# proroklab/magat_pathplanning

Hardware: AMD Instinct MI355X
Metric: agent-steps/s (batched GAT forward) (higher is better)
Workload: dtype f32 in/out, fp32-class arithmetic: convolutions + GAT maps as f16x3 split products on the 16-bit matrix cores with f32 accumulation (the encoder head too, on the layer3 kernel's pooled map; with GAT_MFMA the attention scores and the K-hop aggregation as well), MLPs on f32 MFMA

## Files before the change

include/magat_hip.h:

```cpp
#ifndef MAGAT_HIP_H
#define MAGAT_HIP_H

#include <stddef.h>
#include <stdint.h>

#ifdef __cplusplus
extern "C" {
#endif

#define MAGAT_OK 0
#define MAGAT_ERR_BAD_SHAPE (-1)
#define MAGAT_ERR_UNSUPPORTED (-2)
#define MAGAT_ERR_WORKSPACE (-3)
#define MAGAT_ERR_LAUNCH (-4)
#define MAGAT_ERR_NULL (-5)

#define MAGAT_MODE_KEYQUERY 0
#define MAGAT_MODE_GAT_MODIFIED 1
#define MAGAT_MODE_GAT_ORIGIN 2
#define MAGAT_MODE_GNN 3

int magat_abi_version(void);
int magat_build_flavor(void);
const char* magat_error_string(int code);
// ... 245 lines not shown
#define MAGAT_FORM_GAT_PACK 2
#define MAGAT_FORM_GAT_PERSIST 3
#define MAGAT_FORM_GAT_HSPLIT 4
#define MAGAT_FORM_CHAIN_PERSIST 5
#define MAGAT_FORM_HEAD_COMPRESS 6
#define MAGAT_FORM_GUARD_ONE 7
#define MAGAT_FORM_CSR_FUSED 8
#define MAGAT_FORM_GAT_MID 9
#define MAGAT_FORM_CHAIN_LAT 10
#define MAGAT_FORM_HEAD_LAT 11
#define MAGAT_FORM_GUARD_LAT 12
#define MAGAT_FORM_STEM_LAT 13
#define MAGAT_FORM_ACTIONS_TAIL 14
#define MAGAT_FORM_GNN_DENSE 15
#define MAGAT_FORMS 16
long long magat_form_count(int id);
int magat_form_reset(void);

#ifdef __cplusplus
}
#endif
#endif
```

magat_pathplanning_amd/_native.py:

```python
import ctypes
import os
import threading

PKG = os.path.dirname(os.path.abspath(__file__))
LIB_PATH = os.environ.get("MAGAT_LIB_PATH") or os.path.join(PKG, "lib", "libmagat_hip.so")

MODE_KEYQUERY = 0
MODE_GAT_MODIFIED = 1
MODE_GAT_ORIGIN = 2
MODE_GNN = 3
_MODE_IDS = {"KeyQuery": MODE_KEYQUERY, "GAT_modified": MODE_GAT_MODIFIED, "GAT_origin": MODE_GAT_ORIGIN}
TAGS = {0: "untagged", 1: "conv_first", 2: "layer1.conv1", 3: "layer1.conv2+ds", 4: "layer2.conv1",
        5: "layer2.conv2+ds", 6: "layer3.conv1", 7: "layer3.conv2+ds", 8: "head(avgpool+fc+linear)",
        9: "compressMLP", 10: "gat_maps_gemm", 11: "gat_graph", 12: "actionsMLP", 13: "head_mean",
        14: "gat_pack", 15: "gso_prepare", 16: "gat_prepare", 17: "range_guard", 18: "layer1.conv2+layer2 (fused)", 19: "gat_layer (one launch)", 20: "gso_to_csr", 21: "gat_cast", 22: "layer3 (fused, pooled)", 23: "layer1.conv2+layer2+layer3 (fused, pooled)", 25: "gnn_dense"}
TAG_ACTIONS = 12
FORMS = {"head_longk": 0, "head_splitk": 1, "gat_pack": 2, "gat_persist": 3, "gat_hsplit": 4, "chain_persist": 5,
         "head_compress": 6, "guard_one": 7, "csr_fused": 8, "gat_mid": 9, "chain_lat": 10, "head_lat": 11, "guard_lat": 12, "stem_lat": 13, "actions_tail": 14, "gnn_dense": 15}
TAG_GNN_DENSE = 25

_lock = threading.Lock()
_lib = None


class MagatNativeError(RuntimeError):
    pass


class ConvGemmDesc(ctypes.Structure):
    _fields_ = [("inp", ctypes.c_void_p), ("in2", ctypes.c_void_p), ("wt", ctypes.c_void_p),
                ("bias", ctypes.c_void_p), ("out", ctypes.c_void_p),
                ("in_pix_stride", ctypes.c_int64), ("in2_pix_stride", ctypes.c_int64),
                ("out_pix_stride", ctypes.c_int64), ("M", ctypes.c_int),
# ... 177 lines not shown
```

magat_pathplanning_amd/csrc/gat_mfma.hip:

```cpp
#include <type_traits>

#include "magat_common.h"

namespace {

typedef _Float16 f16x8 __attribute__((ext_vector_type(8)));
typedef _Float16 f16x2 __attribute__((ext_vector_type(2)));

struct GatMfmaParams {
  const float* X;
  const void* S;
  const unsigned* rmask_pre;
  const char* wfrag;
  const float* bias;
  float* Y;
  int B, N, P, ldx, ldy, concat, s_is_f64;
  int Binst;
  int hsplit;
  float* Ypre; int ldpre;
  int* range_flag;
  const float* kconst;
  int origin;
  const float* x_scale;
  long long* dbg;
// ... 67 lines not shown
    const float send = odd ? a[r0] : a[r0 + 1];
    const float recv = dpp_mov<0xB1>(send);
    a[r0] = odd ? recv : a[r0];
    a[r0 + 1] = odd ? a[r0 + 1] : recv;
  }
#pragma unroll
  for (int r0 = 0; r0 < 2; ++r0) {
    const float send = hi ? a[r0] : a[r0 + 2];
    const float recv = dpp_mov<0x4E>(send);
    a[r0] = hi ? recv : a[r0];
    a[r0 + 2] = hi ? a[r0 + 2] : recv;
  }
}

__device__ __forceinline__ uint4 lds128(const char* ptr, int coff) { return *reinterpret_cast<const uint4*>(ptr + coff); }

template <int MT, int KSI, int KT, bool CONCAT, int MODE, bool PACK = false>
__global__ __launch_bounds__(256, 1) void gat_mfma_kernel(const GatMfmaParams p) {
  extern __shared__ __align__(16) char lds[];
  static_assert(!PACK || (MT == 4 && KSI == 2), "PACK: four 32-row slots");
  constexpr int KI = 16 * KSI, SA = 2 * KI + 16;
  constexpr int KIU = PACK ? 128 : KI, SAU = 2 * KIU + 16;
  constexpr int MTS = PACK ? 1 : MT;
  constexpr float kInvScale = 1.f / 256.f;
  const int t = threadIdx.x, lane = t & 63;
  const int w = __builtin_amdgcn_readfirstlane(t >> 6);
  const int fr = lane & 31, h_ = lane >> 5;
  const int N = p.N;
  const int NR = PACK ? 128 : N;
  const int R8 = PACK ? 128 : (N + 7) & ~7;
// ... 26 lines not shown
  auto wr_load = [&](int hd_, int f) __attribute__((always_inline)) {
    int hh = hd_;
    if (f >= FPH) { hh = hd_ + 1 == hhi ? hlo : hd_ + 1; f -= FPH; }
    const int ks = f & 7;
    const char* s = f < 8 ? wl + (size_t)hh * 65536
                          : wl + (size_t)(p.P + hh * KT + (KT - 1 - (f - 8) / 8)) * 65536;
    wr[f & 3][0] = *reinterpret_cast<const uint4*>(s + ks * 2048);
    wr[f & 3][1] = *reinterpret_cast<const uint4*>(s + ks * 2048 + 1024);
  };
#pragma unroll
  for (int f = 0; f < 4; ++f) wr_load(hlo, f);

  for (int b = b0; b < p.B; b += bstride) {
    GM_STAMP(14);
    if (b != b0) GM_SYNC();
    {
      int t = threadIdx.x;
      asm volatile("" : "+v"(t));
      const int lane_ = t & 63;
      const float* Xb = p.X + (long long)b * (PACK ? 4 : 1) * N * p.ldx;
      const unsigned xst = AO + 2048;
      for (int c = w; c * 64 < NR * 32; c += 4) {
        const int ch = c * 64 + lane_;
        const int row = ch >> 5;
        const long long arow = PACK ? (long long)(row >> 5) * N + (row & 31) : row;
        const bool rok = PACK ? ((row & 31) < N && 4 * b + (row >> 5) < p.Binst) : ch < N * 32;
        const float* src = Xb + arow * p.ldx + (ch & 31) * 4;
        const unsigned m0v = __builtin_amdgcn_readfirstlane((unsigned)(uintptr_t)lds + xst + (unsigned)c * 1024u);
        if (rok) asm volatile("s_mov_b32 m0, %1\n\tglobal_load_lds_dwordx4 %0, off" ::"v"(src), "s"(m0v) : "memory", "m0");
      }
      if (!p.rmask_pre) {
        auto stage_pack = [&](auto tag) __attribute__((always_inline)) {
          typedef decltype(tag) ST;
          const int j0 = (lane_ & 31) < N ? (lane_ & 31) : N - 1;
          for (int R0 = w; R0 < 128; R0 += 32) {
            ST v0[8];
#pragma unroll
            for (int r = 0; r < 8; ++r) {
              const int R = R0 + 4 * r, sl = R >> 5, i = min(R & 31, N - 1);
              const int inst = min(4 * b + sl, p.Binst - 1);
              v0[r] = (static_cast<const ST*>(p.S) + (long long)inst * N * N)[(long long)i * N + j0];
            }
#pragma unroll
            for (int r = 0; r < 8; ++r) {
              const int R = R0 + 4 * r, sl = R >> 5, i = R & 31;
              bool f0 = sizeof(ST) == 8 ? fabs((double)v0[r]) > 1e-9 : fabsf((float)v0[r]) > 1e-9f;
              if (MODE == 1 && p.origin) f0 = fabsf((float)v0[r] + ((lane_ & 31) == i ? 1.f : 0.f)) > 1e-9f;
              const unsigned long long k0 = __ballot(f0 && lane_ < N);
              if (lane_ == 0) {
                unsigned* m = reinterpret_cast<unsigned*>(lds + MO) + 4 * R;
                m[0] = (i < N && 4 * b + sl < p.Binst) ? (unsigned)k0 : 0u; m[1] = 0u; m[2] = 0u; m[3] = 0u;
              }
            }
          }
        };
        auto stage = [&](auto tag) {
          typedef decltype(tag) ST;
          const ST* Sp = static_cast<const ST*>(p.S) + (long long)b * N * N;
          const int j0 = lane_ < N ? lane_ : N - 1, j1 = lane_ + 64 < N ? lane_ + 64 : N - 1;
          for (int i0 = w; i0 < N; i0 += 32) {
            ST v0[8], v1[8];
#pragma unroll
            for (int r = 0; r < 8; ++r) {
              const int i = i0 + 4 * r < N ? i0 + 4 * r : N - 1;
              v0[r] = Sp[(long long)i * N + j0];
              v1[r] = Sp[(long long)i * N + j1];
            }
#pragma unroll
            for (int r = 0; r < 8; ++r) {
              const int i = i0 + 4 * r;
              bool f0 = sizeof(ST) == 8 ? fabs((double)v0[r]) > 1e-9 : fabsf((float)v0[r]) > 1e-9f;
              bool f1 = sizeof(ST) == 8 ? fabs((double)v1[r]) > 1e-9 : fabsf((float)v1[r]) > 1e-9f;
              if (MODE == 1 && p.origin) {
                f0 = fabsf((float)v0[r] + (lane_ == i ? 1.f : 0.f)) > 1e-9f;
                f1 = fabsf((float)v1[r] + (lane_ + 64 == i ? 1.f : 0.f)) > 1e-9f;
              }
              const unsigned long long k0 = __ballot(f0 && lane_ < N), k1 = __ballot(f1 && lane_ + 64 < N);
              if (lane_ == 0 && i < N) {
                unsigned* m = reinterpret_cast<unsigned*>(lds + MO) + 4 * i;
                m[0] = (unsigned)k0; m[1] = (unsigned)(k0 >> 32); m[2] = (unsigned)k1; m[3] = (unsigned)(k1 >> 32);
              }
            }
          }
        };
        if constexpr (PACK) {
          if (p.s_is_f64) stage_pack(double{});
          else stage_pack(float{});
        } else {
          if (p.s_is_f64) stage(double{});
          else stage(float{});
        }
      }
      asm volatile("s_waitcnt vmcnt(0)" ::: "memory");
      GM_SYNC();
      for (int idx = t; idx < NR * 16; idx += 256) {
        const int row = idx >> 4, ch = idx & 15;
        f32x4 v0 = *reinterpret_cast<const f32x4*>(lds + xst + idx * 32);
        f32x4 v1 = *reinterpret_cast<const f32x4*>(lds + xst + idx * 32 + 16);
        if (PACK && !((row & 31) < N && 4 * b + (row >> 5) < p.Binst)) v0 = v1 = f32x4{0.f, 0.f, 0.f, 0.f};
        float xv[8] = {v0[0] * xs, v0[1] * xs, v0[2] * xs, v0[3] * xs, v1[0] * xs, v1[1] * xs, v1[2] * xs, v1[3] * xs};
        bool bad = false;
#pragma unroll
        for (int e = 0; e < 8; ++e) bad |= !(fabsf(xv[e]) <= 65504.f);
        if (bad) vmax = __builtin_inff();
        uint4 hi, lo;
        split2v(xv[0], xv[1], hi.x, lo.x, vmax);
        split2v(xv[2], xv[3], hi.y, lo.y, vmax);
        split2v(xv[4], xv[5], hi.z, lo.z, vmax);
        split2v(xv[6], xv[7], hi.w, lo.w, vmax);
        char* dst = lds + (row * 512 + ((ch ^ (row & 15)) << 4));
        *reinterpret_cast<uint4*>(dst) = hi;
        *reinterpret_cast<uint4*>(dst + 256) = lo;
      }
    }
    GM_SYNC();
    GM_STAMP(15);
    unsigned mk[4] = {0u, 0u, 0u, 0u};
    if constexpr (PACK) {
      if (fr < N && 4 * b + w < p.Binst) {
        const unsigned m = p.rmask_pre ? p.rmask_pre[((long long)(4 * b + w) * N + fr) * 4]
                                       : *reinterpret_cast<const unsigned*>(lds + MO + 16 * cw_);
        mk[0] = m >> (4 * h_);
      }
    } else if (cw_ < N) {
      const uint4 m = p.rmask_pre ? *reinterpret_cast<const uint4*>(p.rmask_pre + ((long long)b * N + cw_) * 4)
                                  : *reinterpret_cast<const uint4*>(lds + MO + 16 * cw_);
      mk[0] = m.x >> (4 * h_); mk[1] = m.y >> (4 * h_); mk[2] = m.z >> (4 * h_); mk[3] = m.w >> (4 * h_);
    }
#pragma unroll 1
// ... 386 lines not shown
              }
            }
#ifdef GM_WHATIF_NOYST
            GM_SINK(o[0]);
#else
            if (rok) *dst = o;
#endif
          }
      }
      GM_STAMP(10);
    }
  }
  if (p.range_flag && vmax > 65504.f) atomicOr(p.range_flag, 1);
}

size_t gat_mfma_lds(int N, int ksi) {
  const size_t sa = 2 * 16 * (size_t)ksi + 16, r8 = ((size_t)N + 7) & ~(size_t)7;
  return 2 * (size_t)N * 256 + 2 * r8 * sa + 2 * 128 * sa;
}
constexpr size_t kGatPackLds = 2 * 128 * 256 + 2 * 128 * 80 + 2 * 128 * 272;

int gat_mfma_class(int N) {
  if (N <= 0) return -1;
  const int c = N <= 32 ? 0 : (N <= 64 ? 1 : 2);
  const int ksi = c == 0 ? 2 : (c == 1 ? 4 : 7);
  return (N <= 16 * ksi && gat_mfma_lds(N, ksi) <= 160 * 1024) ? c : -1;
}

template <int KT, int MODE>
int launch_pack(const GatMfmaParams& p, int slot, hipStream_t st) {
// ... 21 lines not shown
int launch(const GatMfmaParams& p, int slot, hipStream_t st) {
  const size_t lds = gat_mfma_lds(p.N, KSI);
  const void* fn = p.concat ? reinterpret_cast<const void*>(&gat_mfma_kernel<MT, KSI, KT, true, MODE>)
                            : reinterpret_cast<const void*>(&gat_mfma_kernel<MT, KSI, KT, false, MODE>);
  if (magat_ensure_dyn_lds(fn, slot + (p.concat ? 0 : 6) + 12 * MODE, lds) != MAGAT_OK) return MAGAT_ERR_LAUNCH;
  int cus = 256, dev = 0;
  if (hipGetDevice(&dev) != hipSuccess ||
      hipDeviceGetAttribute(&cus, hipDeviceAttributeMultiprocessorCount, dev) != hipSuccess || cus <= 0)
    cus = 256;
  GatMfmaParams q = p;
  const long long unsplit = (long long)((p.B + cus - 1) / cus) * (12 + 36 * p.P);
  const long long split = (long long)(((long long)p.B * p.P + cus - 1) / cus) * (12 + 36);
  q.hsplit = ((p.concat || p.Ypre) && p.P > 1 && split < unsplit) ? p.P : 1;
  const long long units = q.hsplit > 1 ? (long long)p.B * p.P : p.B;
  const int blocks = (int)(units < (long long)cus * q.hsplit ? units : (long long)cus * q.hsplit);
  if (q.hsplit > 1) magat_form_note(MAGAT_FORM_GAT_HSPLIT);
  if (units > blocks) magat_form_note(MAGAT_FORM_GAT_PERSIST);
  const int pid = magat_prof_begin(MAGAT_TAG_GAT_LAYER, st);
  if (p.concat) hipLaunchKernelGGL((gat_mfma_kernel<MT, KSI, KT, true, MODE>), dim3(blocks), dim3(256), lds, st, q);
  else {
    hipLaunchKernelGGL((gat_mfma_kernel<MT, KSI, KT, false, MODE>), dim3(blocks), dim3(256), lds, st, q);
    if (q.hsplit > 1 && magat_gat_mean_launch(p.Ypre, p.Y, (long long)p.B * p.N, p.P, 128, p.ldpre, p.ldy, st) != MAGAT_OK) {
      magat_prof_end(pid, st);
      return MAGAT_ERR_LAUNCH;
    }
  }
  magat_prof_end(pid, st);
  return magat_check_launch();
}

template <int MODE>
int launch_class(const GatMfmaParams& p, int K, hipStream_t st) {
  const int cls = gat_mfma_class(p.N);
// ... 46 lines not shown
```

magat_pathplanning_amd/csrc/magat_common.h:

```cpp
#pragma once
#include <hip/hip_runtime.h>
#include <stdint.h>

#include "../../include/magat_hip.h"

typedef float f32x2 __attribute__((ext_vector_type(2)));
typedef float f32x4 __attribute__((ext_vector_type(4)));
typedef float f32x16 __attribute__((ext_vector_type(16)));

#if (defined(MAGAT_WHATIF_NO_W) || defined(MAGAT_WHATIF_NO_LDS) || defined(CSR_WHATIF_NODMA) || defined(CSR_WHATIF_NOLOOP) || defined(CSR_WHATIF_NOIDX) || defined(CSR_WHATIF_NOKLOOP) || defined(CSR_WHATIF_NOSTORE) || \
     defined(GM_WHATIF_NOQW) || defined(GM_WHATIF_NOAW) || defined(GM_WHATIF_NOYST) || defined(FUSED_WHATIF_COALESCED) || defined(FUSED_WHATIF_NOSCALAR)) && !defined(MAGAT_EXPERIMENT_BUILD)
#error "*_WHATIF_* timing switches produce wrong results: they compile only with -DMAGAT_EXPERIMENT_BUILD (see magat_common.h)"
#endif
extern "C" int magat_experiment_mark(void);
#ifdef MAGAT_EXPERIMENT_BUILD
namespace { struct MagatExperimentMark { MagatExperimentMark() { magat_experiment_mark(); } } g_magat_experiment_mark; }
#endif

#define MAGAT_WAVE 64
#define MAGAT_TILE_ROWS 128
__host__ __device__ __forceinline__ long long magat_row_off(long long m, long long ld, long long tile_stride) {
  return (m >> 7) * tile_stride + (m & 127) * ld;
}
#define MAGAT_NUM_XCD 8
// ... 37 lines not shown
                    const float* scales = nullptr, int out_gl = 0, const magat_lat_head* head = nullptr,
                    const magat_lat_guard* guard = nullptr, const magat_lat_stem* stem = nullptr);
int magat_block3(const void* in, float* out, const float* w, const float* b1, const float* b2, int M, int* range_flag,
                 hipStream_t st);
int magat_block_chain(const void* in1, const void* in2, void* out, int out_gl, long long out_pix_stride, long long out_tile,
                      const float* w, const float* bA, const float* bB, const float* bC, int M, int* range_flag,
                      hipStream_t st);
int magat_conv_direct_enabled();
int magat_conv_gemm_chain_f32(const magat_conv_gemm_desc* descs, int n, const int32_t* run_if, int tag, hipStream_t st,
                              int32_t* book = nullptr);

enum MagatOpt {
  MAGAT_OPT_ENC_CHUNK, MAGAT_OPT_CONV_SPLIT, MAGAT_OPT_CONV_PCHAIN,
  MAGAT_OPT_L1_FUSED, MAGAT_OPT_HEAD_SPLITK, MAGAT_OPT_GAT_CHUNK_MB, MAGAT_OPT_GAT_SPLIT, MAGAT_OPT_RANGE_GUARD,
  MAGAT_OPT_BLOCK_FUSED, MAGAT_OPT_CSR_TILED, MAGAT_OPT_HEAD_F16, MAGAT_OPT_GAT_MFMA, MAGAT_OPT_SKINNY, MAGAT_OPT_GAT_PACK,
  MAGAT_OPT_CONV_BNFILL, MAGAT_OPT_HEAD_COMPRESS, MAGAT_OPT_CONV_TM, MAGAT_OPT_CSR_FUSED, MAGAT_OPT_LAT_AGENTS, MAGAT_OPT_GAT_WIDE_FROM, MAGAT_OPT_COUNT
};
int magat_opt(int id);
#define MAGAT_LDS_SLOTS 192
int magat_ensure_dyn_lds(const void* func, int slot, size_t bytes);
enum MagatLdsSlot {
  MAGAT_LDS_GAT16, MAGAT_LDS_GAT32, MAGAT_LDS_GAT64, MAGAT_LDS_GAT128, MAGAT_LDS_GAT256, MAGAT_LDS_L1FUSED,
  MAGAT_LDS_SIM_GSO_T, MAGAT_LDS_SIM_GSO_F, MAGAT_LDS_SIM_MOVE, MAGAT_LDS_BLOCK_A, MAGAT_LDS_BLOCK_B, MAGAT_LDS_BLOCK_C,
  MAGAT_LDS_SIM_CONN, MAGAT_LDS_CONV_FIRST, MAGAT_LDS_CONV_FIRST11, MAGAT_LDS_GSO_STRUCT, MAGAT_LDS_CSR_TILED_A, MAGAT_LDS_CSR_TILED_B, MAGAT_LDS_CSR_TILED_A16, MAGAT_LDS_CSR_TILED_B16,
  MAGAT_LDS_CSR_TILED_A4, MAGAT_LDS_CSR_TILED_B4, MAGAT_LDS_CSR_TILED_A16_4, MAGAT_LDS_CSR_TILED_B16_4, MAGAT_LDS_BLOCK_B4, MAGAT_LDS_BLOCK_FULL, MAGAT_LDS_BLOCK_FULL_P, MAGAT_LDS_BLOCK_FULL_C, MAGAT_LDS_BLOCK_FULL_C4, MAGAT_LDS_BLOCK_FULL_C5,
  MAGAT_LDS_GATM_0,
  MAGAT_LDS_GATM_END = MAGAT_LDS_GATM_0 + 24,
  MAGAT_LDS_STEM8,
  MAGAT_LDS_GATP_0,
  MAGAT_LDS_GATP_END = MAGAT_LDS_GATP_0 + 8,
  MAGAT_LDS_GATS_0,
  MAGAT_LDS_GATS_END = MAGAT_LDS_GATS_0 + 8,
  MAGAT_LDS_CSR_FUSED_A,
  MAGAT_LDS_CSR_FUSED_B = MAGAT_LDS_CSR_FUSED_A + 3,
  MAGAT_LDS_CSR_FUSED_END = MAGAT_LDS_CSR_FUSED_B + 2,
  MAGAT_LDS_GATD_0 = MAGAT_LDS_CSR_FUSED_END,
  MAGAT_LDS_GATD_END = MAGAT_LDS_GATD_0 + 56,
  MAGAT_LDS_BLOCK_LAT, MAGAT_LDS_BLOCK_LAT_H, MAGAT_LDS_BLOCK_LAT_S,
  MAGAT_LDS_GAT_SLIM,
  MAGAT_LDS_GAT_RERUN_S, MAGAT_LDS_GAT_RERUN_S_END = MAGAT_LDS_GAT_RERUN_S + 5,
  MAGAT_LDS_GNND_0,
  MAGAT_LDS_GNND_END = MAGAT_LDS_GNND_0 + 5,
  MAGAT_LDS_END
};
static_assert(MAGAT_LDS_END <= MAGAT_LDS_SLOTS, "LDS attribute slots");

__host__ __device__ inline size_t magat_gat_f16_block_offset(int NC, int G) {
  const size_t a = (((size_t)NC * (G + 1) + 3) & ~(size_t)3) + ((size_t)3 * NC * G + 1) / 2;
  return (a + 3) & ~(size_t)3;
}

__host__ __device__ inline size_t magat_gat_frag_offset(int NC, int G) {
  return (magat_gat_f16_block_offset(NC, G) + (size_t)NC * G + 4 + 3) & ~(size_t)3;
}
__host__ __device__ inline size_t magat_gat_csr_fused_offset(int NC, int G) {
  return (magat_gat_frag_offset(NC, G) + (size_t)NC * G + 3) & ~(size_t)3;
}
// ... 109 lines not shown
```

magat_pathplanning_amd/csrc/options.hip:

```cpp
#include <atomic>
#include <cstdlib>
#include <cstring>
#include <mutex>

#include "magat_common.h"

namespace {

struct OptEntry {
  const char* name;
  int def;
};

const OptEntry kOpts[MAGAT_OPT_COUNT] = {
    {"ENC_CHUNK", 65536},
    {"CONV_SPLIT", 7},
    {"CONV_PCHAIN", 1},
    {"L1_FUSED", 2},
    {"HEAD_SPLITK", 5120},
    {"GAT_CHUNK_MB", 2048},
    {"GAT_SPLIT", 1},
    {"RANGE_GUARD", 1},
    {"BLOCK_FUSED", 2},
    {"CSR_TILED", 3},
    {"HEAD_F16", 1},
    {"GAT_MFMA", 1},
    {"SKINNY", 1},
    {"GAT_PACK", 1},
    {"CONV_BNFILL", 256},
    {"HEAD_COMPRESS", 1},
    {"CONV_TM", 2},
    {"CSR_FUSED", 1},
    {"LAT_AGENTS", 512},
    {"GAT_WIDE_FROM", 103},
};

int g_val[MAGAT_OPT_COUNT];
int g_start[MAGAT_OPT_COUNT];
std::once_flag g_once;

void init_opts() {
  for (int i = 0; i < MAGAT_OPT_COUNT; ++i) {
    g_val[i] = kOpts[i].def;
    char key[64] = "MAGAT_";
    strncat(key, kOpts[i].name, sizeof(key) - 7);
    const char* e = getenv(key);
    if (e && *e) g_val[i] = atoi(e);
    g_start[i] = g_val[i];
  }
// ... 67 lines not shown
```

magat_pathplanning_amd/csrc/profile.hip:

```cpp
#include <algorithm>
#include <atomic>
#include <mutex>
#include <vector>

#include "magat_common.h"

namespace {
struct Span {
  int tag;
  hipEvent_t a, b;
};
bool g_enabled = false;
std::vector<Span> g_pool;
size_t g_used = 0;
double g_total[MAGAT_PROF_TAGS];
long long g_count[MAGAT_PROF_TAGS];
std::mutex g_mu;
constexpr size_t kMaxSpans = 1 << 16;
}

int magat_prof_begin(int tag, hipStream_t st) {
  if (!g_enabled || tag == MAGAT_TAG_UNTAGGED) return -1;
  std::lock_guard<std::mutex> lk(g_mu);
  if (g_used >= kMaxSpans) return -1;
// ... 133 lines not shown
  if (stamps) {
    std::vector<long long> h(2 * (size_t)cus);
    if (hipMemcpy(h.data(), stamps, h.size() * sizeof(long long), hipMemcpyDeviceToHost) != hipSuccess) return MAGAT_ERR_LAUNCH;
    std::vector<double> mhz;
    for (int i = 0; i < cus; ++i)
      if (h[2 * i + 1] > 0) mhz.push_back((double)h[2 * i] / (double)h[2 * i + 1] * 100.0);
    if (mhz.empty()) return MAGAT_ERR_LAUNCH;
    std::sort(mhz.begin(), mhz.end());
    const double med = mhz[mhz.size() / 2];
    if (clock_mhz) *clock_mhz = med;
    if (per_clk) *per_clk = *tflops * 1e12 / (med * 1e6 * (double)cus * 4);
  }
  return MAGAT_OK;
}

namespace { std::atomic<long long> g_forms[MAGAT_FORMS]; }
void magat_form_note(int id) {
  if (id >= 0 && id < MAGAT_FORMS) g_forms[id].fetch_add(1, std::memory_order_relaxed);
}
extern "C" long long magat_form_count(int id) {
  if (id < 0 || id >= MAGAT_FORMS) return -1;
  return g_forms[id].load(std::memory_order_relaxed);
}
extern "C" int magat_form_reset(void) {
  for (int i = 0; i < MAGAT_FORMS; ++i) g_forms[i].store(0, std::memory_order_relaxed);
  return MAGAT_OK;
}
```

Measured before the change: 22.06 million.

## Add 512-thread paired-wavefront GAT kernel splitting map GEMM and tap aggregation

Adds a gat_pair_kernel that runs 8 wavefronts per block. Four wavefronts compute the per-head map GEMM while the other four handle the attention tap and K-hop aggregation, so the two phases can overlap within one block. The staging code is factored into a helper templated on wavefront count so both kernels share it. The kernel is enabled by default for KeyQuery concat layers. This adds register and LDS pressure and more block-level synchronisation.

```diff
diff --git a/include/magat_hip.h b/include/magat_hip.h
--- a/include/magat_hip.h
+++ b/include/magat_hip.h
@@ -283,6 +283,8 @@
 #define MAGAT_FORM_ACTIONS_TAIL 14
 #define MAGAT_FORM_GNN_DENSE 15
 #define MAGAT_FORMS 16
+#define MAGAT_FORM_GAT_PAIR 16
+#define MAGAT_FORMS_ALL 17
 long long magat_form_count(int id);
 int magat_form_reset(void);
 
diff --git a/magat_pathplanning_amd/_native.py b/magat_pathplanning_amd/_native.py
--- a/magat_pathplanning_amd/_native.py
+++ b/magat_pathplanning_amd/_native.py
@@ -16,7 +16,8 @@
         14: "gat_pack", 15: "gso_prepare", 16: "gat_prepare", 17: "range_guard", 18: "layer1.conv2+layer2 (fused)", 19: "gat_layer (one launch)", 20: "gso_to_csr", 21: "gat_cast", 22: "layer3 (fused, pooled)", 23: "layer1.conv2+layer2+layer3 (fused, pooled)", 25: "gnn_dense"}
 TAG_ACTIONS = 12
 FORMS = {"head_longk": 0, "head_splitk": 1, "gat_pack": 2, "gat_persist": 3, "gat_hsplit": 4, "chain_persist": 5,
-         "head_compress": 6, "guard_one": 7, "csr_fused": 8, "gat_mid": 9, "chain_lat": 10, "head_lat": 11, "guard_lat": 12, "stem_lat": 13, "actions_tail": 14, "gnn_dense": 15}
+         "head_compress": 6, "guard_one": 7, "csr_fused": 8, "gat_mid": 9, "chain_lat": 10, "head_lat": 11, "guard_lat": 12, "stem_lat": 13, "actions_tail": 14, "gnn_dense": 15,
+         "gat_pair": 16}
 TAG_GNN_DENSE = 25
 
 _lock = threading.Lock()
diff --git a/magat_pathplanning_amd/csrc/gat_mfma.hip b/magat_pathplanning_amd/csrc/gat_mfma.hip
--- a/magat_pathplanning_amd/csrc/gat_mfma.hip
+++ b/magat_pathplanning_amd/csrc/gat_mfma.hip
@@ -105,6 +105,110 @@
 }
 
 __device__ __forceinline__ uint4 lds128(const char* ptr, int coff) { return *reinterpret_cast<const uint4*>(ptr + coff); }
+
+template <int NW, int MODE, bool PACK>
+__device__ __forceinline__ void gm_stage_instance(const GatMfmaParams& p, char* lds, int b, int w, int N, int NR, unsigned AO,
+                                                  unsigned MO, float xs, float& vmax) {
+  {
+    int t = threadIdx.x;
+    asm volatile("" : "+v"(t));
+    const int lane_ = t & 63;
+    const float* Xb = p.X + (long long)b * (PACK ? 4 : 1) * N * p.ldx;
+    const unsigned xst = AO + 2048;
+    for (int c = w; c * 64 < NR * 32; c += NW) {
+      const int ch = c * 64 + lane_;
+      const int row = ch >> 5;
+      const long long arow = PACK ? (long long)(row >> 5) * N + (row & 31) : row;
+      const bool rok = PACK ? ((row & 31) < N && 4 * b + (row >> 5) < p.Binst) : ch < N * 32;
+      const float* src = Xb + arow * p.ldx + (ch & 31) * 4;
+      const unsigned m0v = __builtin_amdgcn_readfirstlane((unsigned)(uintptr_t)lds + xst + (unsigned)c * 1024u);
+      if (rok) asm volatile("s_mov_b32 m0, %1\n\tglobal_load_lds_dwordx4 %0, off" ::"v"(src), "s"(m0v) : "memory", "m0");
+    }
+    if (!p.rmask_pre) {
+      auto stage_pack = [&](auto tag) __attribute__((always_inline)) {
+        typedef decltype(tag) ST;
+        const int j0 = (lane_ & 31) < N ? (lane_ & 31) : N - 1;
+        for (int R0 = w; R0 < 128; R0 += 8 * NW) {
+          ST v0[8];
+#pragma unroll
+          for (int r = 0; r < 8; ++r) {
+            const int R = R0 + NW * r, sl = R >> 5, i = min(R & 31, N - 1);
+            const int inst = min(4 * b + sl, p.Binst - 1);
+            v0[r] = (static_cast<const ST*>(p.S) + (long long)inst * N * N)[(long long)i * N + j0];
+          }
+#pragma unroll
+          for (int r = 0; r < 8; ++r) {
+            const int R = R0 + NW * r, sl = R >> 5, i = R & 31;
+            bool f0 = sizeof(ST) == 8 ? fabs((double)v0[r]) > 1e-9 : fabsf((float)v0[r]) > 1e-9f;
+            if (MODE == 1 && p.origin) f0 = fabsf((float)v0[r] + ((lane_ & 31) == i ? 1.f : 0.f)) > 1e-9f;
+            const unsigned long long k0 = __ballot(f0 && lane_ < N);
+            if (lane_ == 0) {
+              unsigned* m = reinterpret_cast<unsigned*>(lds + MO) + 4 * R;
+              m[0] = (i < N && 4 * b + sl < p.Binst) ? (unsigned)k0 : 0u; m[1] = 0u; m[2] = 0u; m[3] = 0u;
+            }
+          }
+        }
+      };
+      auto stage = [&](auto tag) {
+        typedef decltype(tag) ST;
+        const ST* Sp = static_cast<const ST*>(p.S) + (long long)b * N * N;
+        const int j0 = lane_ < N ? lane_ : N - 1, j1 = lane_ + 64 < N ? lane_ + 64 : N - 1;
+        for (int i0 = w; i0 < N; i0 += 8 * NW) {
+          ST v0[8], v1[8];
+#pragma unroll
+          for (int r = 0; r < 8; ++r) {
+            const int i = i0 + NW * r < N ? i0 + NW * r : N - 1;
+            v0[r] = Sp[(long long)i * N + j0];
+            v1[r] = Sp[(long long)i * N + j1];
+          }
+#pragma unroll
+          for (int r = 0; r < 8; ++r) {
+            const int i = i0 + NW * r;
+            bool f0 = sizeof(ST) == 8 ? fabs((double)v0[r]) > 1e-9 : fabsf((float)v0[r]) > 1e-9f;
+            bool f1 = sizeof(ST) == 8 ? fabs((double)v1[r]) > 1e-9 : fabsf((float)v1[r]) > 1e-9f;
+            if (MODE == 1 && p.origin) {
+              f0 = fabsf((float)v0[r] + (lane_ == i ? 1.f : 0.f)) > 1e-9f;
+              f1 = fabsf((float)v1[r] + (lane_ + 64 == i ? 1.f : 0.f)) > 1e-9f;
+            }
+            const unsigned long long k0 = __ballot(f0 && lane_ < N), k1 = __ballot(f1 && lane_ + 64 < N);
+            if (lane_ == 0 && i < N) {
+              unsigned* m = reinterpret_cast<unsigned*>(lds + MO) + 4 * i;
+              m[0] = (unsigned)k0; m[1] = (unsigned)(k0 >> 32); m[2] = (unsigned)k1; m[3] = (unsigned)(k1 >> 32);
+            }
+          }
+        }
+      };
+      if constexpr (PACK) {
+        if (p.s_is_f64) stage_pack(double{});
+        else stage_pack(float{});
+      } else {
+        if (p.s_is_f64) stage(double{});
+        else stage(float{});
+      }
+    }
+    asm volatile("s_waitcnt vmcnt(0)" ::: "memory");
+    GM_SYNC();
+    for (int idx = t; idx < NR * 16; idx += 64 * NW) {
+      const int row = idx >> 4, ch = idx & 15;
+      f32x4 v0 = *reinterpret_cast<const f32x4*>(lds + xst + idx * 32);
+      f32x4 v1 = *reinterpret_cast<const f32x4*>(lds + xst + idx * 32 + 16);
+      if (PACK && !((row & 31) < N && 4 * b + (row >> 5) < p.Binst)) v0 = v1 = f32x4{0.f, 0.f, 0.f, 0.f};
+      float xv[8] = {v0[0] * xs, v0[1] * xs, v0[2] * xs, v0[3] * xs, v1[0] * xs, v1[1] * xs, v1[2] * xs, v1[3] * xs};
+      bool bad = false;
+#pragma unroll
+      for (int e = 0; e < 8; ++e) bad |= !(fabsf(xv[e]) <= 65504.f);
+      if (bad) vmax = __builtin_inff();
+      uint4 hi, lo;
+      split2v(xv[0], xv[1], hi.x, lo.x, vmax);
+      split2v(xv[2], xv[3], hi.y, lo.y, vmax);
+      split2v(xv[4], xv[5], hi.z, lo.z, vmax);
+      split2v(xv[6], xv[7], hi.w, lo.w, vmax);
+      char* dst = lds + (row * 512 + ((ch ^ (row & 15)) << 4));
+      *reinterpret_cast<uint4*>(dst) = hi;
+      *reinterpret_cast<uint4*>(dst + 256) = lo;
+    }
+  }
+}
 
 template <int MT, int KSI, int KT, bool CONCAT, int MODE, bool PACK = false>
 __global__ __launch_bounds__(256, 1) void gat_mfma_kernel(const GatMfmaParams p) {
@@ -161,105 +265,7 @@
   for (int b = b0; b < p.B; b += bstride) {
     GM_STAMP(14);
     if (b != b0) GM_SYNC();
-    {
-      int t = threadIdx.x;
-      asm volatile("" : "+v"(t));
-      const int lane_ = t & 63;
-      const float* Xb = p.X + (long long)b * (PACK ? 4 : 1) * N * p.ldx;
-      const unsigned xst = AO + 2048;
-      for (int c = w; c * 64 < NR * 32; c += 4) {
-        const int ch = c * 64 + lane_;
-        const int row = ch >> 5;
-        const long long arow = PACK ? (long long)(row >> 5) * N + (row & 31) : row;
-        const bool rok = PACK ? ((row & 31) < N && 4 * b + (row >> 5) < p.Binst) : ch < N * 32;
-        const float* src = Xb + arow * p.ldx + (ch & 31) * 4;
-        const unsigned m0v = __builtin_amdgcn_readfirstlane((unsigned)(uintptr_t)lds + xst + (unsigned)c * 1024u);
-        if (rok) asm volatile("s_mov_b32 m0, %1\n\tglobal_load_lds_dwordx4 %0, off" ::"v"(src), "s"(m0v) : "memory", "m0");
-      }
-      if (!p.rmask_pre) {
-        auto stage_pack = [&](auto tag) __attribute__((always_inline)) {
-          typedef decltype(tag) ST;
-          const int j0 = (lane_ & 31) < N ? (lane_ & 31) : N - 1;
-          for (int R0 = w; R0 < 128; R0 += 32) {
-            ST v0[8];
-#pragma unroll
-            for (int r = 0; r < 8; ++r) {
-              const int R = R0 + 4 * r, sl = R >> 5, i = min(R & 31, N - 1);
-              const int inst = min(4 * b + sl, p.Binst - 1);
-              v0[r] = (static_cast<const ST*>(p.S) + (long long)inst * N * N)[(long long)i * N + j0];
-            }
-#pragma unroll
-            for (int r = 0; r < 8; ++r) {
-              const int R = R0 + 4 * r, sl = R >> 5, i = R & 31;
-              bool f0 = sizeof(ST) == 8 ? fabs((double)v0[r]) > 1e-9 : fabsf((float)v0[r]) > 1e-9f;
-              if (MODE == 1 && p.origin) f0 = fabsf((float)v0[r] + ((lane_ & 31) == i ? 1.f : 0.f)) > 1e-9f;
-              const unsigned long long k0 = __ballot(f0 && lane_ < N);
-              if (lane_ == 0) {
-                unsigned* m = reinterpret_cast<unsigned*>(lds + MO) + 4 * R;
-                m[0] = (i < N && 4 * b + sl < p.Binst) ? (unsigned)k0 : 0u; m[1] = 0u; m[2] = 0u; m[3] = 0u;
-              }
-            }
-          }
-        };
-        auto stage = [&](auto tag) {
-          typedef decltype(tag) ST;
-          const ST* Sp = static_cast<const ST*>(p.S) + (long long)b * N * N;
-          const int j0 = lane_ < N ? lane_ : N - 1, j1 = lane_ + 64 < N ? lane_ + 64 : N - 1;
-          for (int i0 = w; i0 < N; i0 += 32) {
-            ST v0[8], v1[8];
-#pragma unroll
-            for (int r = 0; r < 8; ++r) {
-              const int i = i0 + 4 * r < N ? i0 + 4 * r : N - 1;
-              v0[r] = Sp[(long long)i * N + j0];
-              v1[r] = Sp[(long long)i * N + j1];
-            }
-#pragma unroll
-            for (int r = 0; r < 8; ++r) {
-              const int i = i0 + 4 * r;
-              bool f0 = sizeof(ST) == 8 ? fabs((double)v0[r]) > 1e-9 : fabsf((float)v0[r]) > 1e-9f;
-              bool f1 = sizeof(ST) == 8 ? fabs((double)v1[r]) > 1e-9 : fabsf((float)v1[r]) > 1e-9f;
-              if (MODE == 1 && p.origin) {
-                f0 = fabsf((float)v0[r] + (lane_ == i ? 1.f : 0.f)) > 1e-9f;
-                f1 = fabsf((float)v1[r] + (lane_ + 64 == i ? 1.f : 0.f)) > 1e-9f;
-              }
-              const unsigned long long k0 = __ballot(f0 && lane_ < N), k1 = __ballot(f1 && lane_ + 64 < N);
-              if (lane_ == 0 && i < N) {
-                unsigned* m = reinterpret_cast<unsigned*>(lds + MO) + 4 * i;
-                m[0] = (unsigned)k0; m[1] = (unsigned)(k0 >> 32); m[2] = (unsigned)k1; m[3] = (unsigned)(k1 >> 32);
-              }
-            }
-          }
-        };
-        if constexpr (PACK) {
-          if (p.s_is_f64) stage_pack(double{});
-          else stage_pack(float{});
-        } else {
-          if (p.s_is_f64) stage(double{});
-          else stage(float{});
-        }
-      }
-      asm volatile("s_waitcnt vmcnt(0)" ::: "memory");
-      GM_SYNC();
-      for (int idx = t; idx < NR * 16; idx += 256) {
-        const int row = idx >> 4, ch = idx & 15;
-        f32x4 v0 = *reinterpret_cast<const f32x4*>(lds + xst + idx * 32);
-        f32x4 v1 = *reinterpret_cast<const f32x4*>(lds + xst + idx * 32 + 16);
-        if (PACK && !((row & 31) < N && 4 * b + (row >> 5) < p.Binst)) v0 = v1 = f32x4{0.f, 0.f, 0.f, 0.f};
-        float xv[8] = {v0[0] * xs, v0[1] * xs, v0[2] * xs, v0[3] * xs, v1[0] * xs, v1[1] * xs, v1[2] * xs, v1[3] * xs};
-        bool bad = false;
-#pragma unroll
-        for (int e = 0; e < 8; ++e) bad |= !(fabsf(xv[e]) <= 65504.f);
-        if (bad) vmax = __builtin_inff();
-        uint4 hi, lo;
-        split2v(xv[0], xv[1], hi.x, lo.x, vmax);
-        split2v(xv[2], xv[3], hi.y, lo.y, vmax);
-        split2v(xv[4], xv[5], hi.z, lo.z, vmax);
-        split2v(xv[6], xv[7], hi.w, lo.w, vmax);
-        char* dst = lds + (row * 512 + ((ch ^ (row & 15)) << 4));
-        *reinterpret_cast<uint4*>(dst) = hi;
-        *reinterpret_cast<uint4*>(dst + 256) = lo;
-      }
-    }
+    gm_stage_instance<4, MODE, PACK>(p, lds, b, w, N, NR, AO, MO, xs, vmax);
     GM_SYNC();
     GM_STAMP(15);
     unsigned mk[4] = {0u, 0u, 0u, 0u};
@@ -676,6 +682,410 @@
   if (p.range_flag && vmax > 65504.f) atomicOr(p.range_flag, 1);
 }
 
+#ifdef MAGAT_DEBUG_HOOKS
+#define GP_STAMP(i) do { if (p.dbg && (threadIdx.x & 63) == 0) p.dbg[((long long)blockIdx.x * 4 + ((threadIdx.x >> 6) & 3)) * 16 + (i)] = (long long)__builtin_readcyclecounter(); } while (0)
+#else
+#define GP_STAMP(i) do { } while (0)
+#endif
+#define GP_VMAX() asm volatile("" : "+v"(vmax))
+template <int MT, int KSI, int KT>
+__global__ __launch_bounds__(512, 1) void gat_pair_kernel(const GatMfmaParams p) {
+  extern __shared__ __align__(16) char lds[];
+  constexpr int KI = 16 * KSI, SA = 2 * KI + 16;
+  constexpr int SAU = SA;
+  constexpr float kInvScale = 1.f / 256.f;
+  const int t = threadIdx.x, lane = t & 63;
+  const int wv = __builtin_amdgcn_readfirstlane(t >> 6);
+  const int w = wv & 3;
+  const bool tapw = wv >= 4;
+  const int fr = lane & 31, h_ = lane >> 5;
+  const int N = p.N;
+  const int NR = N, R8 = (N + 7) & ~7;
+  const unsigned AO = 512u * NR, AP = (unsigned)R8 * SA;
+  const unsigned UO = AO + 2 * AP;
+  constexpr unsigned UP = 128 * SAU;
+  const unsigned MO = AO;
+#define GP_ROWS(rsw, xsw) unsigned rsw[MT], xsw[MT]; { int l_ = lane; asm volatile("" : "+v"(l_)); _Pragma("unroll") \
+    for (int mt_ = 0; mt_ < MT; ++mt_) { const int row_ = min(32 * mt_ + (l_ & 31), N - 1); rsw[mt_] = row_ * 512; \
+      xsw[mt_] = ((l_ >> 5) ^ (row_ & 15)) << 4; } }
+  const int cw_ = 32 * w + fr;
+  auto wlo = [&]() __attribute__((always_inline)) { unsigned o = (unsigned)lane * 16u; asm volatile("" : "+v"(o)); return (unsigned)w * 16384u + o; };
+  float vmax = 0.f;
+  float xs = 1.f;
+  if (p.x_scale) xs = *p.x_scale;
+  if (xs == 0.f) xs = 1.f;
+  const float ixs = 1.f / xs;
+  const int hpw = p.P / p.hsplit, hlo = ((int)blockIdx.x % p.hsplit) * hpw, hhi = hlo + hpw;
+  const int b0 = (int)blockIdx.x / p.hsplit, bstride = (int)gridDim.x / p.hsplit;
+  uint4 wr[4][2];
+
+  if (!tapw) {
+    const bool g2_active = 32 * w < KI;
+    const float kLog2eS = 1.4426950408889634f * ixs * ixs;
+    auto wr_load = [&](int hd_, int f) __attribute__((always_inline)) {
+      int hh = hd_;
+      if (f >= 8) { hh = hd_ + 1 == hhi ? hlo : hd_ + 1; f -= 8; }
+      const char* s = p.wfrag + (wlo() + (unsigned)hh * 65536u + (unsigned)f * 2048u);
+      wr[f & 3][0] = *reinterpret_cast<const uint4*>(s);
+      wr[f & 3][1] = *reinterpret_cast<const uint4*>(s + 1024);
+    };
+#pragma unroll
+    for (int f = 0; f < 4; ++f) wr_load(hlo, f);
+    f32x16 accq[MT];
+    auto g1 = [&](int hd) __attribute__((always_inline)) {
+      GP_ROWS(rsw, xsw)
+#pragma unroll
+      for (int mt = 0; mt < MT; ++mt)
+#pragma unroll
+        for (int r = 0; r < 16; ++r) accq[mt][r] = 0.f;
+      uint4 a[MT][2];
+#pragma unroll
+      for (int mt = 0; mt < MT; ++mt) {
+        const char* ap = lds + (rsw[mt] + xsw[mt]);
+        a[mt][0] = lds128(ap, 0);
+        a[mt][1] = lds128(ap, 256);
+      }
+#pragma unroll
+      for (int ks = 0; ks < 8; ++ks) {
+#pragma unroll
+        for (int q = 0; q < 3; ++q)
+#pragma unroll
+          for (int mt = 0; mt < MT; ++mt) {
+            accq[mt] = mfma16(wr[ks & 3][q == 1 ? 1 : 0], a[mt][q == 2 ? 1 : 0], accq[mt]);
+            if (ks + 1 < 8 && q >= 1)
+              a[mt][q - 1] = lds128(lds + (rsw[mt] + (xsw[mt] ^ (unsigned)((ks + 1) << 5))), 256 * (q - 1));
+          }
+        wr_load(hd, ks + 4);
+        GM_PIN();
+      }
+    };
+    for (int b = b0; b < p.B; b += bstride) {
+      GP_STAMP(14);
+      if (b != b0) GM_SYNC();
+      gm_stage_instance<8, 0, false>(p, lds, b, wv, N, NR, AO, MO, xs, vmax);
+      GM_SYNC();
+      GP_STAMP(15);
+      unsigned mk[4] = {0u, 0u, 0u, 0u};
+      if (cw_ < N) {
+        const uint4 m = p.rmask_pre ? *reinterpret_cast<const uint4*>(p.rmask_pre + ((long long)b * N + cw_) * 4)
+                                    : *reinterpret_cast<const uint4*>(lds + MO + 16 * cw_);
+        mk[0] = m.x >> (4 * h_); mk[1] = m.y >> (4 * h_); mk[2] = m.z >> (4 * h_); mk[3] = m.w >> (4 * h_);
+      }
+      g1(hlo);
+      GP_STAMP(11);
+#pragma unroll 1
+      for (int hd = hlo; hd < hhi; ++hd) {
+        GP_STAMP(0);
+        int cw = cw_, h = h_;
+        asm volatile("" : "+v"(cw), "+v"(h));
+        if (hd > hlo) GM_SYNC();
+        GP_STAMP(1);
+        {
+          const int fr_ = cw & 31;
+          unsigned jb[MT];
+#pragma unroll
+          for (int mt = 0; mt < MT; ++mt) {
+            const int j = 32 * mt + fr_;
+            jb[mt] = UO + (unsigned)(j < R8 ? j : R8) * 512u + 8u * h;
+          }
+          unsigned qx[4];
+#pragma unroll
+          for (int q = 0; q < 4; ++q) {
+            qx[q] = (unsigned)(((4 * w + q) ^ (fr_ & 15)) << 4);
+            asm volatile("" : "+v"(qx[q]));
+          }
+#pragma unroll
+          for (int mt = 0; mt < MT; ++mt)
+#pragma unroll
+            for (int q = 0; q < 4; ++q) {
+              unsigned hq[2], lq[2];
+              const float v01[2] = {mul1(accq[mt][4 * q], kInvScale), mul1(accq[mt][4 * q + 1], kInvScale)};
+              split2v(v01[0], v01[1], hq[0], lq[0], vmax);
+              GP_VMAX();
+              const float v23[2] = {mul1(accq[mt][4 * q + 2], kInvScale), mul1(accq[mt][4 * q + 3], kInvScale)};
+              split2v(v23[0], v23[1], hq[1], lq[1], vmax);
+              GP_VMAX();
+              char* o = lds + (jb[mt] + qx[q]);
+              GM_QW(o, (uint2{hq[0], hq[1]}));
+              GM_QW(o + 256, (uint2{lq[0], lq[1]}));
+            }
+        }
+        GP_STAMP(2);
+        GM_SYNC();
+        GP_STAMP(3);
+        if (g2_active) {
+          GP_ROWS(rsw, xsw)
+          f32x16 acce[MT];
+#pragma unroll
+          for (int mt = 0; mt < MT; ++mt)
+#pragma unroll
+            for (int r = 0; r < 16; ++r) acce[mt][r] = 0.f;
+          {
+            const int rowb = min(32 * w + (cw & 31), N - 1);
+            const unsigned rswb = rowb * 512, xswb = (h ^ (rowb & 15)) << 4;
+            const char* qbase = lds + UO;
+            uint4 a[MT][2], bq[2][2];
+#pragma unroll
+            for (int mt = 0; mt < MT; ++mt) {
+              const char* ap = qbase + (rsw[mt] + xsw[mt]);
+              a[mt][0] = lds128(ap, 0);
+              a[mt][1] = lds128(ap, 256);
+            }
+            {
+              const char* bp = lds + (rswb + xswb);
+              bq[0][0] = lds128(bp, 0);
+              bq[0][1] = lds128(bp, 256);
+            }
+#pragma unroll
+            for (int ks = 0; ks < 8; ++ks) {
+              if (ks + 1 < 8) {
+                const char* bp = lds + (rswb + (xswb ^ (unsigned)((ks + 1) << 5)));
+                bq[(ks + 1) & 1][0] = lds128(bp, 0);
+                bq[(ks + 1) & 1][1] = lds128(bp, 256);
+              }
+#pragma unroll
+              for (int q = 0; q < 3; ++q)
+#pragma unroll
+                for (int mt = 0; mt < MT; ++mt) {
+                  acce[mt] = mfma16(a[mt][q == 2 ? 1 : 0], bq[ks & 1][q == 1 ? 1 : 0], acce[mt]);
+                  if (ks + 1 < 8 && q >= 1)
+                    a[mt][q - 1] = lds128(qbase + (rsw[mt] + (xsw[mt] ^ (unsigned)((ks + 1) << 5))), 256 * (q - 1));
+                }
+              GM_PIN();
+            }
+          }
+          GP_STAMP(12);
+          float mx = -__builtin_inff();
+          unsigned mkl[4] = {mk[0], mk[1], mk[2], mk[3]};
+          asm volatile("" : "+v"(mkl[0]), "+v"(mkl[1]), "+v"(mkl[2]), "+v"(mkl[3]));
+#pragma unroll
+          for (int mt = 0; mt < MT; ++mt)
+#pragma unroll
+            for (int q = 0; q < 4; ++q)
+#pragma unroll
+              for (int e = 0; e < 4; ++e) {
+                const int r = 4 * q + e;
+                const unsigned m = (unsigned)__builtin_amdgcn_sbfe((int)mkl[mt], 8 * (r >> 2) + (r & 3), 1);
+                const float ev = acce[mt][r];
+                const unsigned u = (__builtin_bit_cast(unsigned, ev) & m) | (0xff800000u & ~m);
+                const float em = __builtin_bit_cast(float, u);
+                acce[mt][r] = em;
+                mx = fmaxf(mx, em);
+              }
+          mx = fmaxf(mx, __shfl_xor(mx, 32, 64));
+          const float cexp = mx > -__builtin_inff() ? -mx * kLog2eS : 0.f;
+          float sum = 0.f;
+#pragma unroll
+          for (int mt = 0; mt < MT; ++mt)
+#pragma unroll
+            for (int q = 0; q < 4; ++q)
+#pragma unroll
+              for (int e = 0; e < 4; ++e) {
+                const int r = 4 * q + e;
+                acce[mt][r] = __builtin_amdgcn_exp2f(__builtin_fmaf(acce[mt][r], kLog2eS, cexp));
+                sum += acce[mt][r];
+              }
+          sum += __shfl_xor(sum, 32, 64);
+          const float inv = sum > 0.f ? 256.f / sum : 0.f;
+          GP_STAMP(13);
+          {
+            char* abp = lds + (AO + 4 * h * SA + min(cw, KI + 7) * 2);
+            char* alp = abp + AP;
+#pragma unroll
+            for (int mt = 0; mt < MT; ++mt)
+#pragma unroll
+              for (int q = 0; q < 4; ++q) {
+                unsigned ha[2], la[2];
+                const float v01[2] = {mul1(acce[mt][4 * q], inv), mul1(acce[mt][4 * q + 1], inv)};
+                const float v23[2] = {mul1(acce[mt][4 * q + 2], inv), mul1(acce[mt][4 * q + 3], inv)};
+                split_pair(v01[0], v01[1], ha[0], la[0]);
+                split_pair(v23[0], v23[1], ha[1], la[1]);
+                const int jg = 32 * mt + 8 * q;
+                const unsigned short hv[4] = {(unsigned short)ha[0], (unsigned short)(ha[0] >> 16), (unsigned short)ha[1],
+                                              (unsigned short)(ha[1] >> 16)};
+                const unsigned short lv[4] = {(unsigned short)la[0], (unsigned short)(la[0] >> 16), (unsigned short)la[1],
+                                              (unsigned short)(la[1] >> 16)};
+                if (jg < N) {
+#pragma unroll
+                  for (int e = 0; e < 4; ++e) {
+                    GM_AW(abp + (jg + e) * SA, hv[e]);
+                    GM_AW(alp + (jg + e) * SA, lv[e]);
+                  }
+                }
+              }
+          }
+        }
+        GP_STAMP(4);
+        GM_SYNC();
+        if (hd + 1 < hhi) g1(hd + 1);
+        GP_STAMP(10);
+      }
+    }
+  } else {
+    constexpr int FPH = 8 * KT;
+    const float kOutScale = kInvScale * ixs;
+    const float biasv = p.bias ? p.bias[cw_] : 0.f;
+    auto wr_load = [&](int hd_, int f) __attribute__((always_inline)) {
+      int hh = hd_;
+      if (f >= FPH) { hh = hd_ + 1 == hhi ? hlo : hd_ + 1; f -= FPH; }
+      const int ks = f & 7;
+      const char* s = p.wfrag + (wlo() + (unsigned)(p.P + hh * KT + (KT - 1 - f / 8)) * 65536u + (unsigned)ks * 2048u);
+      wr[f & 3][0] = *reinterpret_cast<const uint4*>(s);
+      wr[f & 3][1] = *reinterpret_cast<const uint4*>(s + 1024);
+    };
+#pragma unroll
+    for (int f = 0; f < 4; ++f) wr_load(hlo, f);
+    for (int b = b0; b < p.B; b += bstride) {
+      if (b != b0) GM_SYNC();
+      gm_stage_instance<8, 0, false>(p, lds, b, wv, N, NR, AO, MO, xs, vmax);
+      GM_SYNC();
+#pragma unroll 1
+      for (int hd = hlo; hd < hhi; ++hd) {
+        int cw = cw_, h = h_;
+        asm volatile("" : "+v"(cw), "+v"(h));
+        f32x16 acc[KT][MT];
+        uint4 a3[MT][2];
+        GP_ROWS(rsw3, xsw3)
+        constexpr int TAP_PER = 3 * MT, TAP_ALL = 8 * TAP_PER;
+        auto tap_load_a1 = [&](int ks, int mt, int pl) __attribute__((always_inline)) {
+          const char* ap = lds + (rsw3[mt] + (xsw3[mt] ^ (unsigned)(ks << 5)));
+          a3[mt][pl] = lds128(ap, 256 * pl);
+        };
+        auto tap_one = [&](int k, int i) __attribute__((always_inline)) {
+          const int ks = i / TAP_PER, r = i % TAP_PER;
+          const int f = 8 * (KT - 1 - k) + ks;
+          if (i == 0) {
+#pragma unroll
+            for (int mt = 0; mt < MT; ++mt) {
+              tap_load_a1(0, mt, 0);
+              tap_load_a1(0, mt, 1);
+#pragma unroll
+              for (int e = 0; e < 16; ++e) acc[k][mt][e] = 0.f;
+            }
+          }
+          const int q = r / MT, mt = r % MT;
+          const int pa = q == 2 ? 1 : 0, pb = q == 1 ? 1 : 0;
+          acc[k][mt] = mfma16(a3[mt][pa], wr[f & 3][pb], acc[k][mt]);
+          if (ks + 1 < 8 && q >= 1) tap_load_a1(ks + 1, mt, q - 1);
+          if (r == TAP_PER - 1) wr_load(hd, f + 4);
+        };
+        auto tap_upto4 = [&](int k, int lo, int hi) __attribute__((always_inline)) {
+#pragma unroll
+          for (int j = 0; j < 4; ++j)
+            if (lo + j < hi) tap_one(k, lo + j);
+        };
+        auto tap_all = [&](int k) __attribute__((always_inline)) {
+#pragma unroll
+          for (int i = 0; i < TAP_ALL; ++i) {
+            tap_one(k, i);
+            if (i % TAP_PER == TAP_PER - 1) GM_PIN();
+          }
+        };
+        if (hd > hlo) GM_SYNC();
+        tap_all(KT - 1);
+        GP_STAMP(5);
+        GM_SYNC();
+        tap_all(KT - 2);
+        GP_STAMP(6);
+        GM_SYNC();
+        GP_STAMP(7);
+        auto hop = [&](auto kc) {
+          constexpr int k = decltype(kc)::value;
+          char* ub = lds + (UO + cw * SAU + h * 8);
+#pragma unroll
+          for (int mt = 0; mt < MT; ++mt)
+#pragma unroll
+            for (int q = 0; q < 4; ++q) {
+              const int i0 = 32 * mt + 8 * q;
+              if (i0 < KI) {
+                constexpr int NG = KI / 8;
+                const int gi = mt * 4 + q;
+                const int u0 = TAP_ALL * gi / NG, u1 = TAP_ALL * (gi + 1) / NG, um = (u0 + u1) / 2;
+                constexpr bool ride = KT == 3 && k == 0;
+                uint2 hi, lo;
+                if constexpr (ride) tap_upto4(0, u0, um);
+                const float v01[2] = {mul1(acc[k + 1][mt][4 * q], kInvScale), mul1(acc[k + 1][mt][4 * q + 1], kInvScale)};
+                split2v(v01[0], v01[1], hi.x, lo.x, vmax);
+                GP_VMAX();
+                GM_PIN();
+                if constexpr (ride) tap_upto4(0, um, u1);
+                const float v23[2] = {mul1(acc[k + 1][mt][4 * q + 2], kInvScale), mul1(acc[k + 1][mt][4 * q + 3], kInvScale)};
+                split2v(v23[0], v23[1], hi.y, lo.y, vmax);
+                GP_VMAX();
+                GM_PIN();
+                *reinterpret_cast<uint2*>(ub + i0 * 2) = hi;
+                *reinterpret_cast<uint2*>(ub + (i0 * 2 + UP)) = lo;
+              }
+            }
+          asm volatile("s_waitcnt lgkmcnt(0)" ::: "memory");
+          unsigned rpa[MT];
+          {
+            int l_ = lane;
+            asm volatile("" : "+v"(l_));
+#pragma unroll
+            for (int mt_ = 0; mt_ < MT; ++mt_) rpa[mt_] = AO + min(32 * mt_ + (l_ & 31), N - 1) * SA + (l_ >> 5) * 16;
+          }
+          const char* up = lds + (UO + cw * SAU + h * 16);
+          const char* apl[MT];
+#pragma unroll
+          for (int mt = 0; mt < MT; ++mt) apl[mt] = lds + rpa[mt];
+          uint4 a[2][MT][2], bu[2][2];
+#pragma unroll
+          for (int mt = 0; mt < MT; ++mt) {
+            a[0][mt][0] = lds128(apl[mt], 0);
+            a[0][mt][1] = lds128(apl[mt] + AP, 0);
+          }
+          bu[0][0] = lds128(up, 0);
+          bu[0][1] = lds128(up, UP);
+#pragma unroll
+          for (int ks = 0; ks < KSI; ++ks) {
+            if (ks + 1 < KSI) {
+#pragma unroll
+              for (int mt = 0; mt < MT; ++mt) {
+                a[(ks + 1) & 1][mt][0] = lds128(apl[mt], (ks + 1) * 32);
+                a[(ks + 1) & 1][mt][1] = lds128(apl[mt] + AP, (ks + 1) * 32);
+              }
+              bu[(ks + 1) & 1][0] = lds128(up, (ks + 1) * 32);
+              bu[(ks + 1) & 1][1] = lds128(up, (ks + 1) * 32 + UP);
+            }
+            mma_step_row<MT>(acc[k], a[ks & 1], bu[ks & 1]);
+            __builtin_amdgcn_sched_barrier(0);
+          }
+        };
+        if constexpr (KT == 3) hop(std::integral_constant<int, 1>{});
+        GP_STAMP(8);
+        hop(std::integral_constant<int, 0>{});
+        GP_STAMP(9);
+        {
+          const int fq = cw & 3;
+          const char* ybase = reinterpret_cast<const char*>(p.Y + (long long)b * N * p.ldy + hd * 128);
+          const unsigned lbyte = (unsigned)((cw & ~3) + (4 * h + fq) * p.ldy) * 4u;
+          const long long rowb = (long long)p.ldy * 4;
+#pragma unroll
+          for (int mt = 0; mt < MT; ++mt)
+#pragma unroll
+            for (int q = 0; q < 4; ++q) {
+              const int jg = 32 * mt + 8 * q;
+              if (jg >= N) break;
+              float v[4];
+#pragma unroll
+              for (int e = 0; e < 4; ++e) v[e] = __builtin_fmaf(acc[0][mt][4 * q + e], kOutScale, biasv);
+              quad_transpose4(v, lane);
+              const bool rok = jg + 4 * h + fq < N;
+              f32x4* dst = reinterpret_cast<f32x4*>(const_cast<char*>(ybase + jg * rowb) + lbyte);
+              f32x4 o = {v[0], v[1], v[2], v[3]};
+#pragma unroll
+              for (int e = 0; e < 4; ++e) o[e] = __builtin_amdgcn_fmed3f(o[e], 0.f, __builtin_inff());
+              if (rok) *dst = o;
+            }
+        }
+      }
+    }
+  }
+  if (p.range_flag && vmax > 65504.f) atomicOr(p.range_flag, 1);
+#undef GP_ROWS
+}
+
 size_t gat_mfma_lds(int N, int ksi) {
   const size_t sa = 2 * 16 * (size_t)ksi + 16, r8 = ((size_t)N + 7) & ~(size_t)7;
   return 2 * (size_t)N * 256 + 2 * r8 * sa + 2 * 128 * sa;
@@ -727,9 +1137,19 @@
   q.hsplit = ((p.concat || p.Ypre) && p.P > 1 && split < unsplit) ? p.P : 1;
   const long long units = q.hsplit > 1 ? (long long)p.B * p.P : p.B;
   const int blocks = (int)(units < (long long)cus * q.hsplit ? units : (long long)cus * q.hsplit);
+  const bool pair = MODE == 0 && p.concat && magat_opt(MAGAT_OPT_GAT_PAIR);
+  if (pair && magat_ensure_dyn_lds(reinterpret_cast<const void*>(&gat_pair_kernel<MT, KSI, KT>),
+                                   MAGAT_LDS_GATPAIR_0 + 2 * (MT == 1 ? 0 : MT / 2) + (KT == 3 ? 0 : 1), lds) != MAGAT_OK)
+    return MAGAT_ERR_LAUNCH;
   if (q.hsplit > 1) magat_form_note(MAGAT_FORM_GAT_HSPLIT);
   if (units > blocks) magat_form_note(MAGAT_FORM_GAT_PERSIST);
+  if (pair) magat_form_note(MAGAT_FORM_GAT_PAIR);
   const int pid = magat_prof_begin(MAGAT_TAG_GAT_LAYER, st);
+  if (pair) {
+    hipLaunchKernelGGL((gat_pair_kernel<MT, KSI, KT>), dim3(blocks), dim3(512), lds, st, q);
+    magat_prof_end(pid, st);
+    return magat_check_launch();
+  }
   if (p.concat) hipLaunchKernelGGL((gat_mfma_kernel<MT, KSI, KT, true, MODE>), dim3(blocks), dim3(256), lds, st, q);
   else {
     hipLaunchKernelGGL((gat_mfma_kernel<MT, KSI, KT, false, MODE>), dim3(blocks), dim3(256), lds, st, q);
diff --git a/magat_pathplanning_amd/csrc/magat_common.h b/magat_pathplanning_amd/csrc/magat_common.h
--- a/magat_pathplanning_amd/csrc/magat_common.h
+++ b/magat_pathplanning_amd/csrc/magat_common.h
@@ -75,7 +75,8 @@
   MAGAT_OPT_ENC_CHUNK, MAGAT_OPT_CONV_SPLIT, MAGAT_OPT_CONV_PCHAIN,
   MAGAT_OPT_L1_FUSED, MAGAT_OPT_HEAD_SPLITK, MAGAT_OPT_GAT_CHUNK_MB, MAGAT_OPT_GAT_SPLIT, MAGAT_OPT_RANGE_GUARD,
   MAGAT_OPT_BLOCK_FUSED, MAGAT_OPT_CSR_TILED, MAGAT_OPT_HEAD_F16, MAGAT_OPT_GAT_MFMA, MAGAT_OPT_SKINNY, MAGAT_OPT_GAT_PACK,
-  MAGAT_OPT_CONV_BNFILL, MAGAT_OPT_HEAD_COMPRESS, MAGAT_OPT_CONV_TM, MAGAT_OPT_CSR_FUSED, MAGAT_OPT_LAT_AGENTS, MAGAT_OPT_GAT_WIDE_FROM, MAGAT_OPT_COUNT
+  MAGAT_OPT_CONV_BNFILL, MAGAT_OPT_HEAD_COMPRESS, MAGAT_OPT_CONV_TM, MAGAT_OPT_CSR_FUSED, MAGAT_OPT_LAT_AGENTS, MAGAT_OPT_GAT_WIDE_FROM, MAGAT_OPT_GAT_PAIR,
+  MAGAT_OPT_COUNT
 };
 int magat_opt(int id);
 #define MAGAT_LDS_SLOTS 192
@@ -102,6 +103,8 @@
   MAGAT_LDS_GAT_RERUN_S, MAGAT_LDS_GAT_RERUN_S_END = MAGAT_LDS_GAT_RERUN_S + 5,
   MAGAT_LDS_GNND_0,
   MAGAT_LDS_GNND_END = MAGAT_LDS_GNND_0 + 5,
+  MAGAT_LDS_GATPAIR_0,
+  MAGAT_LDS_GATPAIR_END = MAGAT_LDS_GATPAIR_0 + 6,
   MAGAT_LDS_END
 };
 static_assert(MAGAT_LDS_END <= MAGAT_LDS_SLOTS, "LDS attribute slots");
diff --git a/magat_pathplanning_amd/csrc/options.hip b/magat_pathplanning_amd/csrc/options.hip
--- a/magat_pathplanning_amd/csrc/options.hip
+++ b/magat_pathplanning_amd/csrc/options.hip
@@ -33,6 +33,7 @@
     {"CSR_FUSED", 1},
     {"LAT_AGENTS", 512},
     {"GAT_WIDE_FROM", 103},
+    {"GAT_PAIR", 1},
 };
 
 int g_val[MAGAT_OPT_COUNT];
diff --git a/magat_pathplanning_amd/csrc/profile.hip b/magat_pathplanning_amd/csrc/profile.hip
--- a/magat_pathplanning_amd/csrc/profile.hip
+++ b/magat_pathplanning_amd/csrc/profile.hip
@@ -171,15 +171,15 @@
   return MAGAT_OK;
 }
 
-namespace { std::atomic<long long> g_forms[MAGAT_FORMS]; }
+namespace { std::atomic<long long> g_forms[MAGAT_FORMS_ALL]; }
 void magat_form_note(int id) {
-  if (id >= 0 && id < MAGAT_FORMS) g_forms[id].fetch_add(1, std::memory_order_relaxed);
+  if (id >= 0 && id < MAGAT_FORMS_ALL) g_forms[id].fetch_add(1, std::memory_order_relaxed);
 }
 extern "C" long long magat_form_count(int id) {
-  if (id < 0 || id >= MAGAT_FORMS) return -1;
+  if (id < 0 || id >= MAGAT_FORMS_ALL) return -1;
   return g_forms[id].load(std::memory_order_relaxed);
 }
 extern "C" int magat_form_reset(void) {
-  for (int i = 0; i < MAGAT_FORMS; ++i) g_forms[i].store(0, std::memory_order_relaxed);
+  for (int i = 0; i < MAGAT_FORMS_ALL; ++i) g_forms[i].store(0, std::memory_order_relaxed);
   return MAGAT_OK;
 }
```

New measurement: 22.19 million (median of 6 runs). About the same (+0.6%).
